# Ushio/2dGaussianSplatting

Measured on AMD Instinct MI355X. Metric: train iters/sec (fwd+bwd+Adam) + PSNR vs ref; 4K img, 1M splats, higher is better.
Workload: dtype f32; 1 GPU; 4096x4096 synthetic RGB, 1000000 Gaussians, fp32 (BASELINE.json configs[3]); width=4096, height=4096, n_splats=1000000, parallelism=rowslab1, rebin_interval=0, exchange_requested=none, exchange=none

## Files before the change

### 2dgaussiansplatting_amd/csrc/s2d_api.hip

```cpp
#include "../../include/splat2d.h"
#include "../../include/splat2d_test.h"

#include <algorithm>
#include <vector>
#include <climits>
#include <cmath>
#include <cstdarg>
#include <cstddef>
#include <cstdio>
#include <cstring>
#include <cstdlib>
#include <new>

#include "s2d_device.h"
#include "s2d_density.h"
#include "s2d_lists.h"
#include "s2d_owned.h"
#include "s2d_state.h"

using namespace s2d;

struct s2d_ctx {
    s2d_config cfg{};
    Geometry g{};
    int n = 0;
    int device = 0;
    hipStream_t stream = nullptr;
    bool own_stream = false;
    float lr = 0.05f;

    SplatState state;
    DevBuf<float> d_grads_own;
    float* d_grads = nullptr;
    DevBuf<ProjRec> d_proj;
    DevBuf<TileRect> d_rects;
    DevBuf<uint32_t> d_counts;
    DevBuf<uint32_t> d_offsets;
    DevBuf<uint32_t> d_scan_temp;
    TileLists lists;
    DevBuf<unsigned long long> d_wave_masks;
    DevBuf<uint32_t> d_exec_list;
    DevBuf<uint32_t> d_tile_exec;
    DevBuf<uint32_t> d_retire_hint;
    bool deterministic = false;
    DevBuf<float> d_det_data;
    DevBuf<uint32_t> d_det_stamp;
    DevBuf<uint32_t> d_det_touched;
    uint32_t det_epoch = 0;
    bool ref_order = false;
    uint64_t ref_max_bytes = 32ull << 30;
    DevBuf<float> d_ref_terms;
    DevBuf<float> d_pixel_sqerr;
    uint64_t chunk_pairs = 1ull << 30;
    std::vector<int> chunks;
    int chunks_used = 0;
    int chunk_built = -1;
    DevBuf<float4> d_state;
    DevBuf<uint32_t> d_chunk_alive;
    HostBuf<uint32_t> h_chunk_alive;
    bool lists_valid = false;
    bool proj_fresh = false;
    Event ev_flag;
    int check_seq = 1;
    HostBuf<int> h_rebin_stamp;
    int rebin_interval = 1;
    int since_rebin = 0;
    float margin = 0.0f;
    DevBuf<uint8_t> d_image0;
    DevBuf<uint8_t> d_ref;
    bool half_images = false;
    size_t pixel_bytes = sizeof(float4);
    SqerrTrace trace;
    DensityStats density;
    DevBuf<DeviceStatus> d_status;
    DevBuf<PairCounters> d_counters;
    HostBuf<DeviceStatus> h_status;

    float beta1t = 1.0f, beta2t = 1.0f;
    int iterations = 0;
    float good_beta1t = 1.0f, good_beta2t = 1.0f;
    int good_iterations = 0;
    bool have_target = false;
    bool have_forward = false;
    bool have_backward = false;
    char err[512] = {0};
    S2D_LOCAL ~s2d_ctx() = default;
};

namespace {

int fail(s2d_ctx* c, int code, const char* fmt, ...)
{
    if (c) {
        va_list ap;
        va_start(ap, fmt);
        vsnprintf(c->err, sizeof(c->err), fmt, ap);
        va_end(ap);
    }
    return code;
}

#define S2D_HIP(c, expr)                                                                              \
    do {                                                                                              \
        hipError_t e_ = (expr);                                                                       \
        if (e_ != hipSuccess)                                                                         \
            return fail((c), S2D_E_HIP, "%s failed: %s (%s:%d)", #expr, hipGetErrorString(e_), __FILE__, __LINE__); \
    } while (0)

struct IdleAtExit {
    hipStream_t stream;
    ~IdleAtExit() { (void)hipStreamSynchronize(stream); }
};

int use_device(s2d_ctx* c)
{
    S2D_HIP(c, hipSetDevice(c->device));
    return S2D_OK;
}

int ensure_pair_capacity(s2d_ctx* c, uint64_t need)
{
    if (need <= c->lists.capacity()) return S2D_OK;
    if (need >= 0xFFFF0000ull) return fail(c, S2D_E_NOMEM, "tile lists need %llu pairs (> 2^32)", (unsigned long long)need);
    uint64_t cap = std::max<uint64_t>(need + need / 4 + 4096, 1 << 16);
    if (cap > 0xFFFF0000ull) cap = 0xFFFF0000ull;
    if (c->ref_order) {
        const uint64_t per_slot = (uint64_t)kRefTermsStride * sizeof(float);
        if (cap * per_slot > c->ref_max_bytes) cap = std::max<uint64_t>(need, 1 << 16);
        if (cap * per_slot > c->ref_max_bytes)
            return fail(c, S2D_E_NOMEM, "the term scratch of S2D_CFG_REFERENCE_ORDER needs %llu bytes for %llu (tile, splat) pairs, "
                        "S2D_REFERENCE_ORDER_MAX_BYTES allows %llu", (unsigned long long)(cap * per_slot), (unsigned long long)cap,
                        (unsigned long long)c->ref_max_bytes);
    }
    S2D_HIP(c, hipStreamSynchronize(c->stream));
    c->lists.release_pairs();
    c->d_wave_masks.release(), c->d_exec_list.release(), c->d_det_data.release(), c->d_det_stamp.release();
    c->d_ref_terms.release();
    S2D_HIP(c, c->lists.alloc_pairs(cap));
    const auto hand_over = [&]() -> int {
        S2D_HIP(c, c->d_wave_masks.alloc((size_t)cap * 4));
        S2D_HIP(c, c->d_exec_list.alloc((size_t)cap));
        if (c->deterministic) S2D_HIP(c, c->d_det_data.alloc((size_t)cap * kDetStride));
        if (c->ref_order) S2D_HIP(c, c->d_ref_terms.alloc((size_t)cap * kRefTermsStride));
        if (c->deterministic || c->ref_order) {
            S2D_HIP(c, c->d_det_stamp.alloc((size_t)cap));
            S2D_HIP(c, hipMemsetAsync(c->d_det_stamp, 0, (size_t)cap * sizeof(uint32_t), c->stream));
        }
        return S2D_OK;
    };
    const int rc = hand_over();
    if (rc != S2D_OK) c->lists.release_pairs();
    return rc;
}

int rebuild_lists(s2d_ctx* c, int first = 0, int count = -1, bool* need_ranges = nullptr)
{
    const int n = count < 0 ? c->n : count;
    uint64_t total = 0;
    c->lists_valid = false;
    S2D_HIP(c, c->lists.count(ListInput{c->d_rects + first, c->d_counts + first, c->d_offsets + first, first, n, c->d_scan_temp},
                              c->stream, &total));
    if (need_ranges) *need_ranges = total > c->chunk_pairs;
    if (need_ranges && *need_ranges) return S2D_OK;
    if (total >= 0xFFFF0000ull)
        return fail(c, S2D_E_NOMEM, "the tile lists of splats %d..%d need more than 2^32 - 65536 (tile, splat) pairs", first, first + n - 1);
    if (int rc = ensure_pair_capacity(c, total)) return rc;
    S2D_HIP(c, c->lists.finish(c->stream));
    c->lists_valid = count < 0;
    c->since_rebin = 0;
    return S2D_OK;
}

RasterArgs raster_args(const s2d_ctx* c, int first = 0, int count = -1)
{
    RasterArgs a;
    a.tile_off = c->lists.tile_off(); a.list = c->lists.list(); a.wave_masks = c->d_wave_masks;
    a.exec_list = c->d_exec_list; a.tile_exec = c->d_tile_exec; a.retire_hint = c->d_retire_hint;
    a.proj = c->d_proj + first; a.grads = c->d_grads + (size_t)first * 9;
    a.image0 = c->d_image0; a.image_ref = c->d_ref; a.tile_sqerr = c->trace.tile_sqerr();
    a.g = c->g; a.status = c->d_status; a.iteration = c->iterations; a.counters = c->d_counters;
    a.state = c->d_state; a.any_alive = c->d_chunk_alive;
    if (c->deterministic)
        a.det = DetGather{c->d_rects + first, c->d_offsets + first, c->d_counts + first, c->d_det_data, c->d_det_stamp,
                          c->d_det_touched + first, 0u, count < 0 ? c->n : count};
    a.half_images = c->half_images; a.count = (c->cfg.flags & S2D_CFG_COUNT_PAIRS) != 0; a.exact_exp = (c->cfg.flags & S2D_CFG_EXACT_EXP) != 0;
    return a;
}

ProjectArgs project_args(const s2d_ctx* c, const float* splats, int mode)
{
    ProjectArgs a;
    a.splats = splats; a.held = c->state.held(); a.n = c->n; a.g = c->g; a.mode = mode; a.proj = c->d_proj; a.counts = c->d_counts;
    a.check = ContainmentCheck{c->d_rects, c->d_status, mode ? c->check_seq : 0, mode ? (int*)c->h_rebin_stamp : nullptr};
    if (mode == 0) a.margin = c->margin, a.row_counts = c->lists.row_counts();
    return a;
}

AdamArgs adam_args(s2d_ctx* c, uint32_t flags, bool project)
{
    const SplatState::AdamStep st = c->state.adam_step();
    AdamArgs a;
    a.splats = st.arrays.splats; a.adams = st.arrays.adams; a.grads = c->d_grads; a.compact = st.compact;
    a.held_ids = st.held_ids; a.held_count = st.held_count; a.dormant = st.dormant; a.n = c->n; a.g = c->g;
    a.beta1t = c->beta1t; a.beta2t = c->beta2t; a.lr = c->lr; a.iteration = c->iterations;
    a.mode = ((flags & S2D_STEP_OPTIMIZE_OPACITY) ? 1 : 0) | ((c->cfg.flags & S2D_CFG_ADAM_FP32) ? 2 : 0);
    a.proj = project ? (ProjRec*)c->d_proj : nullptr;
    a.check = ContainmentCheck{c->d_rects, c->d_status, c->check_seq, c->h_rebin_stamp};
    a.sq = c->trace.take_for_adam();
    return a;
}

void with_backward_walk(s2d_ctx* c, RasterArgs& a, bool need_opacity_grad)
{
    a.need_opacity_grad = need_opacity_grad;
    if (c->deterministic) a.det.now = ++c->det_epoch;
}

int plan_chunks(s2d_ctx* c)
{
    std::vector<uint32_t> cnt((size_t)c->n);
    S2D_HIP(c, hipMemcpyAsync(cnt.data(), c->d_counts, cnt.size() * sizeof(uint32_t), hipMemcpyDeviceToHost, c->stream));
    S2D_HIP(c, hipStreamSynchronize(c->stream));
    c->chunks.assign(1, 0);
    uint64_t acc = 0;
    for (int i = 0; i < c->n; i++) {
        if (acc > 0 && acc + cnt[(size_t)i] > c->chunk_pairs) {
            c->chunks.push_back(i);
            acc = 0;
        }
        acc += cnt[(size_t)i];
    }
    c->chunks.push_back(c->n);
    if (!c->d_state) S2D_HIP(c, c->d_state.alloc((size_t)c->g.W * (size_t)(c->g.row_end - c->g.row_begin)));
    if (!c->d_chunk_alive) S2D_HIP(c, c->d_chunk_alive.alloc(1));
    S2D_HIP(c, c->h_chunk_alive.alloc(1, hipHostMallocDefault));
    return S2D_OK;
}

int build_chunk(s2d_ctx* c, int k, RasterArgs* a)
{
    const int first = c->chunks[(size_t)k], count = c->chunks[(size_t)k + 1] - first;
    if (c->chunk_built != k) {
        c->chunk_built = -1;
        if (int rc = rebuild_lists(c, first, count)) return rc;
        c->chunk_built = k;
    }
    *a = raster_args(c, first, count); a->first = k == 0;
    return S2D_OK;
}

int chunked_forward(s2d_ctx* c)
{
    const int K = (int)c->chunks.size() - 1;
    c->chunks_used = 0;
    c->chunk_built = -1;
    for (int k = 0; k < K; k++) {
        RasterArgs a;
        if (int rc = build_chunk(c, k, &a)) return rc;
        S2D_HIP(c, hipMemsetAsync(c->d_chunk_alive, 0, sizeof(uint32_t), c->stream));
        S2D_HIP(c, launch_raster(RasterPass::ForwardRange, a, c->stream));
        c->chunks_used = k + 1;
        if (k + 1 < K) {
            S2D_HIP(c, hipMemcpyAsync(c->h_chunk_alive, c->d_chunk_alive, sizeof(uint32_t), hipMemcpyDeviceToHost, c->stream));
            S2D_HIP(c, hipStreamSynchronize(c->stream));
            if (*(volatile uint32_t*)c->h_chunk_alive == 0u) break;
        }
    }
    return S2D_OK;
}

int chunked_backward(s2d_ctx* c, bool need_opacity_grad, const float4* upstream = nullptr)
{
    for (int k = 0; k < c->chunks_used; k++) {
        RasterArgs a;
        if (int rc = build_chunk(c, k, &a)) return rc;
        a.upstream = upstream;
        with_backward_walk(c, a, need_opacity_grad);
        S2D_HIP(c, launch_raster(RasterPass::BackwardRange, a, c->stream));
    }
    return S2D_OK;
}

struct RasterJob {
    bool fused = false;
    bool need_opacity_grad = true;
    bool write_image = true;
};

int launch_job(s2d_ctx* c, bool optimistic, const RasterJob& job)
{
    RasterArgs a = raster_args(c);
    a.abort_stamp = optimistic ? c->check_seq : 0;
    if (job.fused) {
        with_backward_walk(c, a, job.need_opacity_grad);
        a.write_image = job.write_image;
        if (c->trace.plan(true, true) == SqerrBy::PassItself) a.sq = c->trace.job(c->iterations);
    }
    if (c->ref_order && a.exact_exp)
        S2D_HIP(c, launch_reference_forward_exact(a, c->stream));
    else
        S2D_HIP(c, launch_raster(job.fused ? RasterPass::Fused : RasterPass::Forward, a, c->stream));
    return S2D_OK;
}

enum class Stale { Frames, Projection, Lists };

void invalidate(s2d_ctx* c, Stale reach)
{
    c->have_forward = c->have_backward = false;
    if (reach >= Stale::Projection) c->proj_fresh = false;
    if (reach >= Stale::Lists) c->lists_valid = false;
}

constexpr DeviceStatus kFreshStatus{0, INT_MAX, 0, 0};

int splats_replaced(s2d_ctx* c)
{
    S2D_HIP(c, c->state.written(true));
    S2D_HIP(c, hipMemcpyAsync(c->d_status, &kFreshStatus, sizeof(DeviceStatus), hipMemcpyHostToDevice, c->stream));
    invalidate(c, Stale::Lists);
    return S2D_OK;
}

int queue_project(s2d_ctx* c, int mode)
{
    SplatState::Arrays now;
    S2D_HIP(c, c->state.current(&now));
    S2D_HIP(c, launch_project(project_args(c, now.splats, mode), c->stream));
    return S2D_OK;
}

int queue_raster(s2d_ctx* c, const RasterJob& job)
{
    if (!c->have_target) return fail(c, S2D_E_STATE, "no target image set (s2d_set_target)");
    const bool scheduled = !c->lists_valid || c->rebin_interval <= 1 || c->since_rebin >= c->rebin_interval;
    bool rebuild = scheduled;
    bool stored_image0 = !job.fused || job.write_image;
    if (!scheduled) {
        if (!c->proj_fresh) {
            c->check_seq++;
            if (int rc = queue_project(c, 1)) return rc;
            S2D_HIP(c, hipEventRecord(c->ev_flag, c->stream));
            c->proj_fresh = true;
        }
        if (int rc = launch_job(c, true, job)) return rc;
        S2D_HIP(c, hipEventSynchronize(c->ev_flag));
        rebuild = *(volatile int*)c->h_rebin_stamp == c->check_seq;
    }
    if (rebuild) {
        int rc = queue_project(c, 0);
        if (rc != S2D_OK) return rc;
        c->chunks.clear();
        bool need_ranges = false;
        if ((rc = rebuild_lists(c, 0, -1, &need_ranges)) != S2D_OK) return rc;
        if (need_ranges && (c->cfg.flags & S2D_CFG_COUNT_PAIRS))
            return fail(c, S2D_E_NOMEM, "pair counting (S2D_CFG_COUNT_PAIRS) is not available for scenes beyond %llu (tile, splat) pairs",
                        (unsigned long long)c->chunk_pairs);
        if (need_ranges && c->ref_order)
            return fail(c, S2D_E_NOMEM, "reference order (S2D_CFG_REFERENCE_ORDER) is not available for scenes beyond %llu (tile, splat) pairs",
                        (unsigned long long)c->chunk_pairs);
        c->proj_fresh = true;
        c->check_seq++;
        if (need_ranges) {
            if ((rc = plan_chunks(c)) != S2D_OK) return rc;
            if ((rc = chunked_forward(c)) != S2D_OK) return rc;
            if (job.fused && (rc = chunked_backward(c, job.need_opacity_grad)) != S2D_OK) return rc;
            stored_image0 = true;
        } else if ((rc = launch_job(c, false, job)) != S2D_OK) {
            return rc;
        }
    }
    c->have_forward = stored_image0;
    c->have_backward = false;
    return S2D_OK;
}

int queue_forward(s2d_ctx* c) { return queue_raster(c, RasterJob{}); }

int backward_queued(s2d_ctx* c, SqerrBy by)
{
    c->have_backward = true;
    S2D_HIP(c, c->trace.record(c->iterations, by));
    return S2D_OK;
}

int queue_backward_reference(s2d_ctx* c, bool need_opacity_grad, const float4* upstream)
{
    RasterArgs a = raster_args(c);
    a.upstream = upstream;
    a.need_opacity_grad = need_opacity_grad;
    SplatState::Arrays now;
    S2D_HIP(c, c->state.current(&now));
    RefOrder ro;
    ro.splats = now.splats; ro.rects = c->d_rects; ro.offsets = c->d_offsets; ro.counts = c->d_counts; ro.n = c->n;
    ro.terms = c->d_ref_terms; ro.stamp = c->d_det_stamp; ro.capacity = (uint32_t)c->lists.capacity(); ro.now = ++c->det_epoch;
    ro.pixel_sqerr = c->d_pixel_sqerr;
    S2D_HIP(c, launch_reference_backward(a, ro, c->stream));
    if (upstream) return backward_queued(c, SqerrBy::NoLoss);
    S2D_HIP(c, launch_reference_sqerr(c->d_pixel_sqerr, (size_t)c->g.W * (size_t)(c->g.row_end - c->g.row_begin),
                                      c->trace.job(c->iterations).out, c->d_status, c->iterations, c->stream));
    return backward_queued(c, SqerrBy::PassItself);
}

int density_refused(s2d_ctx* c)
{
    if ((c->cfg.flags & (S2D_CFG_COUNT_PAIRS | S2D_CFG_EXACT_EXP)) || c->ref_order)
        return fail(c, S2D_E_INVALID, "density statistics are not available with S2D_CFG_COUNT_PAIRS, S2D_CFG_EXACT_EXP or "
                    "S2D_CFG_REFERENCE_ORDER");
    return S2D_OK;
}

int queue_backward(s2d_ctx* c, bool need_opacity_grad, const float4* upstream = nullptr, bool density = false)
{
    if (!c->have_forward) return fail(c, S2D_E_STATE, "the backward pass needs s2d_forward on the current parameters");
    if (c->ref_order) return queue_backward_reference(c, need_opacity_grad, upstream);
    if (density && !c->chunks.empty())
        return fail(c, S2D_E_NOMEM, "density statistics are not available for scenes beyond %llu (tile, splat) pairs (index-range rendering)",
                    (unsigned long long)c->chunk_pairs);
    if (!c->chunks.empty()) {
        if (int rc = chunked_backward(c, need_opacity_grad, upstream)) return rc;
    } else {
        RasterArgs a = raster_args(c);
        a.upstream = upstream;
        if (density) S2D_HIP(c, c->density.next_pass(&a.density));
        with_backward_walk(c, a, need_opacity_grad);
        S2D_HIP(c, launch_raster(RasterPass::Backward, a, c->stream));
    }
    return backward_queued(c, upstream ? SqerrBy::NoLoss : c->trace.plan(false, false));
}

int queue_forward_backward(s2d_ctx* c, bool need_opacity_grad, bool write_image)
{
    if ((c->cfg.flags & S2D_CFG_COUNT_PAIRS) || c->ref_order) {
        if (int rc = queue_forward(c)) return rc;
        return queue_backward(c, need_opacity_grad);
    }
    RasterJob job;
    job.fused = true;
    job.need_opacity_grad = need_opacity_grad;
    job.write_image = write_image;
    if (int rc = queue_raster(c, job)) return rc;
    return backward_queued(c, c->trace.plan(true, c->chunks.empty()));
}

int queue_adam(s2d_ctx* c, uint32_t flags)
{
    c->beta1t *= kAdamBeta1;
    c->beta2t *= kAdamBeta2;
    const bool fuse = c->lists_valid && c->rebin_interval > 1;
    if (fuse) c->check_seq++;
    S2D_HIP(c, launch_adam(adam_args(c, flags, fuse), c->stream));
    if (fuse) S2D_HIP(c, hipEventRecord(c->ev_flag, c->stream));
    invalidate(c, Stale::Projection);
    c->proj_fresh = fuse;
    c->iterations++;
    c->since_rebin++;
    return S2D_OK;
}

int queue_status_read(s2d_ctx* c)
{
    S2D_HIP(c, hipMemcpyAsync(c->h_status, c->d_status, sizeof(DeviceStatus), hipMemcpyDeviceToHost, c->stream));
    return S2D_OK;
}

int judge_status(s2d_ctx* c)
{
    if (c->h_status->nonfinite) {
        const int k = c->h_status->first_nonfinite_iter;
        if (k >= c->good_iterations && k < c->iterations) {
            float b1 = c->good_beta1t, b2 = c->good_beta2t;
            for (int i = c->good_iterations; i <= k; i++) { b1 *= kAdamBeta1; b2 *= kAdamBeta2; }
            c->beta1t = b1;
            c->beta2t = b2;
            c->iterations = k + 1;
            invalidate(c, Stale::Frames);
        }
        return fail(c, S2D_E_NONFINITE, "non-finite parameter after iteration %d (the reference abort()s, main.cpp:752-785)", k);
    }
    c->good_beta1t = c->beta1t;
    c->good_beta2t = c->beta2t;
    c->good_iterations = c->iterations;
    return S2D_OK;
}

int check_status(s2d_ctx* c)
{
    if (int rc = queue_status_read(c)) return rc;
    S2D_HIP(c, hipStreamSynchronize(c->stream));
    return judge_status(c);
}

double mse_norm(const s2d_ctx* c) { return (double)((long long)c->g.H * c->g.W * 3); }

size_t slab_pixels(const s2d_ctx* c) { return (size_t)c->g.W * (size_t)(c->g.row_end - c->g.row_begin); }

}

extern "C" {

int s2d_abi_version(void) { return S2D_ABI_VERSION; }

int s2d_create(const s2d_config* cfg, s2d_ctx** out)
{
    if (!cfg || !out || cfg->struct_size != sizeof(s2d_config)) return S2D_E_INVALID;
    *out = nullptr;
    if (cfg->width <= 0 || cfg->height <= 0 || cfg->n_splats < 0 || cfg->width > 65536 || cfg->height > 65536)
        return S2D_E_INVALID;
    int rb = cfg->row_begin, re = cfg->row_end;
// ... 702 lines not shown
```

### 2dgaussiansplatting_amd/csrc/s2d_device.h

```cpp
#pragma once

#include <hip/hip_runtime.h>
#include <stdint.h>

#include "s2d_math.h"

namespace s2d {

struct alignas(16) ProjRec {
    float4 q0, q1, q2, q3;
};
static_assert(sizeof(ProjRec) == 64, "ProjRec must be 64 bytes");

struct TileRect {
    uint16_t tx0, tx1, ty0, ty1;
};

struct Geometry {
    int W, H;
    int row_begin;
    int row_end;
    int tiles_x;
    int trow0;
    int tiles_y;
    int num_tiles;
};

struct PairCounters {
    unsigned long long fwd_visited, fwd_active, bwd_visited, bwd_active, fwd_staged, bwd_staged, fwd_wave_execs,
        bwd_wave_execs;
    unsigned long long bwd_lane_hist[65];
    unsigned long long fwd_staged_hit;
    unsigned long long fwd_rows_hit;
    unsigned long long bwd_quadrant_execs;
};

struct DeviceStatus {
    int nonfinite;
    int first_nonfinite_iter;
    int rebin_needed;
    int pad;
};

struct SqerrJob {
    const double* tile_sqerr;
    int num_tiles;
    double* out;
    double* scratch;
};

#if defined(__HIPCC__)
__device__ __forceinline__ float as_f(int v) { return __int_as_float(v); }

__device__ __forceinline__ void raise_rebin(DeviceStatus* status, int stamp, int* host_stamp)
{
    __hip_atomic_store(&status->rebin_needed, stamp, __ATOMIC_RELAXED, __HIP_MEMORY_SCOPE_AGENT);
    if (host_stamp) __hip_atomic_store(host_stamp, stamp, __ATOMIC_RELAXED, __HIP_MEMORY_SCOPE_SYSTEM);
}

__device__ __forceinline__ ProjRec pack_proj(const Projected& p)
{
    ProjRec rec;
    rec.q0 = make_float4(p.pos_x, p.pos_y, p.a, p.b);
    rec.q1 = make_float4(p.d, p.col_r, p.col_g, p.col_b);
    rec.q2 = make_float4(p.opacity, as_f(p.begY), as_f(p.endY), p.cosT);
    const float sx2 = p.sx * p.sx, sy2 = p.sy * p.sy;
    rec.q3 = make_float4(p.sinT, 1.0f / (sx2 * p.sx), 1.0f / (sy2 * p.sy), (sx2 - sy2) / (sx2 * p.sy * p.sy));
    return rec;
}

__device__ __forceinline__ bool tile_rect_of(const Projected& p, const Geometry& g, float margin, TileRect* r)
{
    const int m = (int)margin;
    long long y0 = (long long)p.begY - m, y1 = (long long)p.endY + m;
    if (p.begY == (int)0x80000000u || p.endY == (int)0x80000000u) return false;
    if (y0 < g.row_begin) y0 = g.row_begin;
    if (y1 > g.row_end - 1) y1 = g.row_end - 1;
    if (y0 > y1) return false;
    float xlo = p.pos_x - p.hx - 1.0f - margin;
    float xhi = p.pos_x + p.hx + 1.0f + margin;
    if (!(xlo <= xhi)) return false;
    if (xhi < 0.0f || xlo > (float)(g.W - 1)) return false;
    xlo = fmaxf(xlo, 0.0f);
    xhi = fminf(xhi, (float)(g.W - 1));
    r->tx0 = (uint16_t)((int)xlo >> 4);
    r->tx1 = (uint16_t)((int)xhi >> 4);
    r->ty0 = (uint16_t)(((int)y0 >> 4) - g.trow0);
    r->ty1 = (uint16_t)(((int)y1 >> 4) - g.trow0);
    return true;
}

__device__ __forceinline__ bool rect_still_covers(const Projected& p, const Geometry& g, const TileRect& binned)
{
    TileRect r;
    if (!tile_rect_of(p, g, 0.0f, &r)) return true;
    return binned.tx0 <= binned.tx1 && r.tx0 >= binned.tx0 && r.tx1 <= binned.tx1 && r.ty0 >= binned.ty0 &&
           r.ty1 <= binned.ty1;
}
#endif

constexpr float kAnisoMargin = 1.0f;
constexpr int kRasterBatch = 64;
constexpr int kSortItemsPerThread = 16;
constexpr int kSortBlock = 256;
constexpr int kSortItemsPerBlock = kSortBlock * kSortItemsPerThread;
constexpr int kScanItemsPerThread = 8;
constexpr int kScanBlock = 256;
constexpr int kScanItemsPerBlock = kScanBlock * kScanItemsPerThread;

size_t scan_temp_words(int64_t n);
hipError_t exclusive_scan_u32(const uint32_t* in, uint32_t* out, int64_t n, uint32_t* temp, uint32_t* total_dev,
                              hipStream_t stream, uint32_t* total_host_mapped = nullptr);
size_t sort_temp_words(int64_t n);
hipError_t sort_pairs_u32(uint32_t* keys_a, uint32_t* vals_a, uint32_t* keys_b, uint32_t* vals_b, int64_t n,
                          int key_bits, uint32_t* temp, uint32_t** keys_out, uint32_t** vals_out, uint32_t* tile_first,
                          hipStream_t stream);
size_t tile_first_temp_words(int num_keys);
hipError_t launch_tile_offsets_from_first(const uint32_t* tile_first, int num_keys, uint32_t total, uint32_t* temp,
                                          uint32_t* tile_off, hipStream_t stream);

struct ContainmentCheck {
    TileRect* rects = nullptr;
    DeviceStatus* status = nullptr;
    int stamp = 0;
    int* host_stamp = nullptr;
};

struct ProjectArgs {
    const float* splats = nullptr;
    const uint8_t* held = nullptr;
    int n = 0;
    Geometry g{};
    float margin = 0.0f;
    int mode = 0;
    ProjRec* proj = nullptr;
    uint32_t* counts = nullptr;
    uint32_t* row_counts = nullptr;
    ContainmentCheck check{};
};
hipError_t launch_project(const ProjectArgs& a, hipStream_t stream);
hipError_t launch_emit_row_entries(const TileRect* rects, const uint32_t* row_offsets, const uint32_t* row_counts, int n,
                                   uint32_t* keys, uint32_t* vals, uint32_t capacity, hipStream_t stream);
hipError_t launch_emit_pairs(const TileRect* rects, const uint32_t* offsets, const uint32_t* counts, int n, Geometry g,
                             uint32_t* keys, uint32_t* vals, uint32_t capacity, hipStream_t stream);
hipError_t launch_tile_offsets(const uint32_t* sorted_keys, uint32_t num_pairs, int num_tiles,
                               uint32_t* tile_off, hipStream_t stream, uint32_t key_mask = 0xFFFFFFFFu);

constexpr int kTlMaxColumns = 512;
constexpr int kTlRowBits = 12;
size_t tl_workspace_words(uint64_t entries, int tiles_x, int tiles_y);
hipError_t launch_tile_lists_from_rows(const uint32_t* entries, const uint32_t* entry_keys, uint64_t num_entries, const uint32_t* row_off,
                                       Geometry g, uint32_t* chunk_base, uint32_t* workspace, uint32_t* tile_off, uint32_t* list,
                                       hipStream_t stream);

constexpr int kDetStride = 12;
struct DetGather {
    const TileRect* rects;
    const uint32_t* offsets;
    const uint32_t* counts;
    float* data;
    uint32_t* stamp;
    uint32_t* touched;
    uint32_t now;
    int n;
};
enum class RasterPass {
    Forward,
    Backward,
    Fused,
    ForwardRange,
    BackwardRange,
};
struct RasterArgs {
    const uint32_t* tile_off = nullptr;
    const uint32_t* list = nullptr;
    const ProjRec* proj = nullptr;
    void* image0 = nullptr;
    const void* image_ref = nullptr;
    const float4* upstream = nullptr;
    float* density = nullptr;
    unsigned long long* wave_masks = nullptr;
    uint32_t* exec_list = nullptr;
    uint32_t* tile_exec = nullptr;
    uint32_t* retire_hint = nullptr;
    float* grads = nullptr;
    double* tile_sqerr = nullptr;
    Geometry g{};
    const DeviceStatus* status = nullptr;
    int iteration = 0;
    int abort_stamp = 0;
    PairCounters* counters = nullptr;
    float4* state = nullptr;
    bool first = false;
    uint32_t* any_alive = nullptr;
    bool write_image = false;
    SqerrJob sq{};
    DetGather det{};
    bool half_images = false;
    bool count = false;
    bool exact_exp = false;
    bool need_opacity_grad = false;
};
hipError_t launch_raster(RasterPass pass, const RasterArgs& a, hipStream_t stream);
constexpr int kRefTermsStride = 9 * kTile * kTile;
struct RefOrder {
    const float* splats = nullptr;
    const TileRect* rects = nullptr;
    const uint32_t* offsets = nullptr;
    const uint32_t* counts = nullptr;
    int n = 0;
    float* terms = nullptr;
    uint32_t* stamp = nullptr;
    uint32_t capacity = 0;
    uint32_t now = 0;
    float* pixel_sqerr = nullptr;
};
hipError_t launch_reference_backward(const RasterArgs& a, const RefOrder& ro, hipStream_t stream);
hipError_t launch_reference_forward_exact(const RasterArgs& a, hipStream_t stream);
hipError_t launch_reference_sqerr(const float* pixel_sqerr, size_t pixels, double* out, const DeviceStatus* status, int iteration,
                                  hipStream_t stream);
hipError_t launch_halo_masks(const float* splats, const uint8_t* held, int n, int world, const int* row_bounds, float margin,
                             uint32_t* masks, hipStream_t stream);
hipError_t launch_halo_commit(const uint32_t* masks, int n, int rank, uint8_t* held, uint32_t* ids, uint32_t* count_dev,
                              uint32_t* scan_work, uint32_t* scan_temp, hipStream_t stream);
hipError_t launch_compact_copy(float* base, int w, const uint32_t* ids, const uint32_t* count_dev, int n, float* compact, bool to_compact,
                               hipStream_t stream);
hipError_t launch_rows_gather(const float* base, int w, const int* ids, int count, int n, float* out, hipStream_t stream);
hipError_t launch_rows_scatter(float* base, int w, const int* ids, int count, int n, const float* in, hipStream_t stream);
hipError_t launch_grads_combine(float* grads, const int* rows, int n_rows, const int* src, int world, const float* recv,
                                int n, hipStream_t stream);
constexpr int kSqerrChunks = 64;
constexpr int kSqerrScratchDoubles = kSqerrChunks + 1;
constexpr int kSqerrSmallTiles = 1024;


#if defined(__HIPCC__)
__device__ __forceinline__ double block_sum_256(double v, double* s)
{
#pragma unroll
    for (int d = 32; d >= 1; d >>= 1) v += __shfl_down(v, d, 64);
    if ((threadIdx.x & 63) == 0) s[threadIdx.x >> 6] = v;
    __syncthreads();
    const double r = ((s[0] + s[1]) + s[2]) + s[3];
    __syncthreads();
    return r;
}

__device__ __forceinline__ double sqerr_sum_small(const double* tile_sqerr, int num_tiles, double* s4)
{
    double a = 0.0;
    for (int i = (int)threadIdx.x; i < num_tiles; i += 256)
        a += __hip_atomic_load(tile_sqerr + i, __ATOMIC_RELAXED, __HIP_MEMORY_SCOPE_AGENT);
    return block_sum_256(a, s4);
}

__device__ __forceinline__ void sqerr_reduce(const double* __restrict__ tile_sqerr, int num_tiles, double* __restrict__ out,
                                             double* scratch, int first_chunk, int chunk_stride)
{
    __shared__ double s[4];
    __shared__ bool last;
    if (num_tiles <= kSqerrSmallTiles) {
        if (first_chunk != 0) return;
        const double total = sqerr_sum_small(tile_sqerr, num_tiles, s);
        if (threadIdx.x == 0) *out = total;
        return;
    }
    unsigned long long* ticket = reinterpret_cast<unsigned long long*>(scratch + kSqerrChunks);
    const int chunk = (num_tiles + kSqerrChunks - 1) / kSqerrChunks;
    unsigned long long mine = 0;
    for (int b = first_chunk; b < kSqerrChunks; b += chunk_stride, mine++) {
        const int beg = b * chunk, end = min(beg + chunk, num_tiles);
        double a0 = 0, a1 = 0, a2 = 0, a3 = 0;
        for (int i = beg + (int)threadIdx.x; i < end; i += 1024) {
            a0 += tile_sqerr[i];
            if (i + 256 < end) a1 += tile_sqerr[i + 256];
            if (i + 512 < end) a2 += tile_sqerr[i + 512];
            if (i + 768 < end) a3 += tile_sqerr[i + 768];
        }
        const double part = block_sum_256((a0 + a1) + (a2 + a3), s);
        if (threadIdx.x == 0) __hip_atomic_store(scratch + b, part, __ATOMIC_RELAXED, __HIP_MEMORY_SCOPE_AGENT);
    }
    if (threadIdx.x == 0) {
        __threadfence();
        last = mine != 0 && atomicAdd(ticket, mine) + mine == (unsigned long long)kSqerrChunks;
    }
    __syncthreads();
    if (!last) return;
    __threadfence();
    const double p = threadIdx.x < kSqerrChunks
                         ? __hip_atomic_load(scratch + threadIdx.x, __ATOMIC_RELAXED, __HIP_MEMORY_SCOPE_AGENT)
                         : 0.0;
    const double total = block_sum_256(p, s);
    if (threadIdx.x == 0) {
        *out = total;
        *ticket = 0ull;
    }
}
#endif
hipError_t launch_sqerr_finalize(SqerrJob sq, const DeviceStatus* status, int iteration, hipStream_t stream);

hipError_t launch_init_splats(float* splats, float* adams, int n, int W, int H, hipStream_t stream);
struct AdamArgs {
    float* splats = nullptr;
    float* adams = nullptr;
    float* grads = nullptr;
    const uint32_t* held_ids = nullptr;
    const uint32_t* held_count = nullptr;
    int n = 0;
    Geometry g{};
    float beta1t = 1.0f, beta2t = 1.0f, lr = 0.0f;
    int mode = 0;
    int iteration = 0;
    ProjRec* proj = nullptr;
    ContainmentCheck check{};
    uint8_t* dormant = nullptr;
    SqerrJob sq{};
    bool compact = false;
};
hipError_t launch_adam(const AdamArgs& a, hipStream_t stream);
hipError_t launch_synthetic_target(void* image_ref, bool half_images, int W, int H, int row_begin, int row_end, hipStream_t stream);
hipError_t launch_convert_f32_to_f16(const float4* src, void* dst, size_t pixels, hipStream_t stream);
hipError_t launch_convert_f16_to_f32(const void* src, float4* dst, size_t pixels, hipStream_t stream);
hipError_t launch_test_sincos(const float* x, int n, float* s, float* c, hipStream_t stream);

}
```

### 2dgaussiansplatting_amd/csrc/s2d_optim.hip

```cpp
#include <hip/hip_fp16.h>

#include "s2d_device.h"

namespace s2d {

__global__ __launch_bounds__(256) void init_splats_kernel(float* __restrict__ splats, float* __restrict__ adams, int n,
                                                          int W, int H)
{
    const int i = blockIdx.x * blockDim.x + threadIdx.x;
    if (i >= n) return;
    const Splat s = init_splat((uint32_t)i, W, H);
    float* o = splats + (size_t)i * 9;
    o[0] = s.pos_x; o[1] = s.pos_y; o[2] = s.sx; o[3] = s.sy; o[4] = s.rot;
    o[5] = s.col_r; o[6] = s.col_g; o[7] = s.col_b; o[8] = s.opacity;
    float* a = adams + (size_t)i * 18;
#pragma unroll
    for (int k = 0; k < 18; k++) a[k] = 0.0f;
}

__device__ __forceinline__ bool finite_f32(float x) { return (f32_bits(x) & 0x7f800000u) != 0x7f800000u; }

__device__ __forceinline__ void adam_update_one(float (&v)[9], float (&mv)[18], const float (&gr)[9], int W, int H, float beta1t,
                                                float beta2t, float lr, int mode, int iteration, DeviceStatus* status)
{
#pragma unroll
    for (int k = 0; k < 9; k++)
        if (k < 8 || (mode & 1))
            v[k] = adam_optimize(mv[2 * k], mv[2 * k + 1], v[k], gr[k], lr, beta1t, beta2t, (mode & 2) != 0);
    v[0] = glm_clamp(v[0], 0.0f, (float)W - 1.0f);
    v[1] = glm_clamp(v[1], 0.0f, (float)H - 1.0f);
    v[2] = glm_clamp(v[2], 1.0f, 1024.0f);
    v[3] = glm_clamp(v[3], 1.0f, 1024.0f);
    v[5] = glm_clamp(v[5], 0.0f, 1.0f);
    v[6] = glm_clamp(v[6], 0.0f, 1.0f);
    v[7] = glm_clamp(v[7], 0.0f, 1.0f);
    v[8] = glm_clamp(v[8], 0.1f, 1.0f);
    const bool ok = finite_f32(v[5]) && finite_f32(v[6]) && finite_f32(v[7]) && finite_f32(v[2]) &&
                    finite_f32(v[3]) && finite_f32(v[4]) && finite_f32(v[0]);
    if (!ok) {
        atomicOr(&status->nonfinite, 1);
        atomicMin(&status->first_nonfinite_iter, iteration);
    }
}

__device__ __forceinline__ void project_updated(const float (&v)[9], int i, const Geometry& g, DeviceStatus* status,
                                                ProjRec* __restrict__ proj, const TileRect* __restrict__ rects,
                                                int check_stamp, int* __restrict__ host_stamp)
{
    const float reach = 3.0f * fmaxf(v[2], v[3]) + 2.0f;
    if (v[1] + reach < (float)g.row_begin || v[1] - reach > (float)g.row_end) {
        proj[i].q2 = make_float4(v[8], as_f(1), as_f(0), 0.0f);
        return;
    }
    Splat s;
    s.pos_x = v[0]; s.pos_y = v[1]; s.sx = v[2]; s.sy = v[3]; s.rot = v[4];
    s.col_r = v[5]; s.col_g = v[6]; s.col_b = v[7]; s.opacity = v[8];
    const Projected p = project(s);
    proj[i] = pack_proj(p);
    if (!rect_still_covers(p, g, rects[i])) raise_rebin(status, check_stamp, host_stamp);
}

__device__ __forceinline__ bool adam_prologue(const DeviceStatus* status, int iteration, const SqerrJob& sq)
{
    if (status->first_nonfinite_iter < iteration) return false;
    if (sq.tile_sqerr != nullptr && blockIdx.x < (unsigned)kSqerrChunks)
        sqerr_reduce(sq.tile_sqerr, sq.num_tiles, sq.out, sq.scratch, (int)blockIdx.x, min((int)gridDim.x, kSqerrChunks));
    return true;
}

template <int WIDTH>
__device__ __forceinline__ void lds_fill(float* lds, const float* __restrict__ src, const uint32_t* s_ids, int base, int cnt)
{
    const int floats = cnt * WIDTH;
    if (s_ids == nullptr) {
        const float* p = src + (size_t)base * WIDTH;
        const int vec = floats >> 2;
        for (int q = threadIdx.x; q < vec; q += 256) reinterpret_cast<float4*>(lds)[q] = reinterpret_cast<const float4*>(p)[q];
        for (int q = (vec << 2) + threadIdx.x; q < floats; q += 256) lds[q] = p[q];
    } else {
        for (int q = threadIdx.x; q < floats; q += 256) lds[q] = src[(size_t)s_ids[q / WIDTH] * WIDTH + q % WIDTH];
    }
}

template <int WIDTH>
__device__ __forceinline__ void lds_drain(float* __restrict__ dst, const float* lds, const uint32_t* s_ids, int base, int cnt)
{
    const int floats = cnt * WIDTH;
    if (s_ids == nullptr) {
        float* p = dst + (size_t)base * WIDTH;
        const int vec = floats >> 2;
        for (int q = threadIdx.x; q < vec; q += 256) reinterpret_cast<float4*>(p)[q] = reinterpret_cast<const float4*>(lds)[q];
        for (int q = (vec << 2) + threadIdx.x; q < floats; q += 256) p[q] = lds[q];
    } else {
        for (int q = threadIdx.x; q < floats; q += 256) dst[(size_t)s_ids[q / WIDTH] * WIDTH + q % WIDTH] = lds[q];
    }
}

__global__ __launch_bounds__(256) void adam_kernel(float* __restrict__ splats, float* __restrict__ adams,
                                                   float* __restrict__ grads, const uint32_t* __restrict__ held_ids,
                                                   const uint32_t* __restrict__ held_count, int n, Geometry g,
                                                   float beta1t, float beta2t, float lr, int mode, int iteration,
                                                   DeviceStatus* __restrict__ status, ProjRec* __restrict__ proj,
                                                   const TileRect* __restrict__ rects, int check_stamp,
                                                   int* __restrict__ host_stamp, uint8_t* __restrict__ dormant, SqerrJob sq,
                                                   int compact)
{
    __shared__ __attribute__((aligned(16))) float buf[256 * 18];
    __shared__ uint32_t s_idbuf[256];
    if (!adam_prologue(status, iteration, sq)) return;
    const int total = held_ids ? (int)min(*held_count, (uint32_t)n) : n;
    const int base = blockIdx.x * 256, cnt = min(256, total - base), t = threadIdx.x;
    if (cnt <= 0) return;
    const bool mine = t < cnt;
    const uint32_t* s_ids = nullptr;
    int i = base + t;
    if (held_ids) {
        if (mine) {
            i = (int)held_ids[base + t];
            s_idbuf[t] = (uint32_t)i;
        }
        s_ids = s_idbuf;
        __syncthreads();
    }
    const uint32_t* const s_ids_state = compact ? nullptr : s_ids;
    float v[9], mv[18], gr[9];
    lds_fill<9>(buf, grads, s_ids, base, cnt);
    __syncthreads();
#pragma unroll
    for (int k = 0; k < 9; k++) gr[k] = mine ? buf[t * 9 + k] : 0.0f;
    bool live = false;
    if (mine) {
#pragma unroll
        for (int k = 0; k < 9; k++) live = live || (f32_bits(gr[k]) != 0u);
        if (!live) live = dormant == nullptr || dormant[i] == 0;
    }
    if (!__syncthreads_or(live)) return;
    for (int q = t; q < 256 * 9 / 4; q += 256) reinterpret_cast<float4*>(buf)[q] = make_float4(0.f, 0.f, 0.f, 0.f);
    __syncthreads();
    lds_drain<9>(grads, buf, s_ids, base, cnt);
    __syncthreads();
    lds_fill<9>(buf, splats, s_ids_state, base, cnt);
    __syncthreads();
#pragma unroll
    for (int k = 0; k < 9; k++) v[k] = mine ? buf[t * 9 + k] : 0.0f;
    __syncthreads();
    lds_fill<18>(buf, adams, s_ids_state, base, cnt);
    __syncthreads();
#pragma unroll
    for (int k = 0; k < 18; k++) mv[k] = mine ? buf[t * 18 + k] : 0.0f;
    if (mine) {
        adam_update_one(v, mv, gr, g.W, g.H, beta1t, beta2t, lr, mode, iteration, status);
        if (dormant) {
            uint32_t any = 0u;
#pragma unroll
            for (int k = 0; k < 18; k++) any |= f32_bits(mv[k]);
            dormant[i] = any == 0u ? 1 : 0;
        }
#pragma unroll
        for (int k = 0; k < 18; k++) buf[t * 18 + k] = mv[k];
    }
    __syncthreads();
    lds_drain<18>(adams, buf, s_ids_state, base, cnt);
    __syncthreads();
    if (mine) {
#pragma unroll
        for (int k = 0; k < 9; k++) buf[t * 9 + k] = v[k];
    }
    __syncthreads();
    lds_drain<9>(splats, buf, s_ids_state, base, cnt);
    if (proj && mine) project_updated(v, i, g, status, proj, rects, check_stamp, host_stamp);
}

__device__ __forceinline__ uint2 pack_half4(float4 c)
{
    const __half2 a = __floats2half2_rn(c.x, c.y), b = __floats2half2_rn(c.z, c.w);
    uint2 v;
    v.x = *reinterpret_cast<const uint32_t*>(&a);
    v.y = *reinterpret_cast<const uint32_t*>(&b);
    return v;
}

template <bool HALF>
__global__ __launch_bounds__(256) void synthetic_target_kernel(void* __restrict__ image_ref, int W, int H, int row_begin,
                                                               int row_end)
{
    const int x = blockIdx.x * blockDim.x + threadIdx.x;
    const int y = row_begin + (int)blockIdx.y;
    if (x >= W || y >= row_end) return;
    const float fx = (float)x / (float)W;
    const float4 c = make_float4(fx, 1.0f - fx, (float)y / (float)H, 1.0f);
    const size_t at = (size_t)(y - row_begin) * W + x;
    if (HALF) reinterpret_cast<uint2*>(image_ref)[at] = pack_half4(c);
    else reinterpret_cast<float4*>(image_ref)[at] = c;
}

__global__ __launch_bounds__(256) void convert_f32_to_f16_kernel(const float4* __restrict__ src, uint2* __restrict__ dst,
                                                                 size_t pixels)
{
    const size_t i = (size_t)blockIdx.x * blockDim.x + threadIdx.x;
    if (i < pixels) dst[i] = pack_half4(src[i]);
}

__global__ __launch_bounds__(256) void convert_f16_to_f32_kernel(const uint2* __restrict__ src, float4* __restrict__ dst,
                                                                 size_t pixels)
{
    const size_t i = (size_t)blockIdx.x * blockDim.x + threadIdx.x;
    if (i >= pixels) return;
    const uint2 v = src[i];
    const float2 a = __half22float2(*reinterpret_cast<const __half2*>(&v.x));
    const float2 b = __half22float2(*reinterpret_cast<const __half2*>(&v.y));
    dst[i] = make_float4(a.x, a.y, b.x, b.y);
}

__global__ __launch_bounds__(256) void test_sincos_kernel(const float* __restrict__ x, int n, float* __restrict__ s,
                                                          float* __restrict__ c)
{
    const int i = blockIdx.x * blockDim.x + threadIdx.x;
    if (i >= n) return;
    s[i] = sinf_ref(x[i]);
    c[i] = cosf_ref(x[i]);
}

hipError_t launch_init_splats(float* splats, float* adams, int n, int W, int H, hipStream_t stream)
{
    if (n <= 0) return hipSuccess;
    hipLaunchKernelGGL(init_splats_kernel, dim3((n + 255) / 256), dim3(256), 0, stream, splats, adams, n, W, H);
    return hipGetLastError();
}

hipError_t launch_adam(const AdamArgs& a, hipStream_t stream)
{
    if (a.n <= 0) return hipSuccess;
    hipLaunchKernelGGL(adam_kernel, dim3((a.n + 255) / 256), dim3(256), 0, stream, a.splats, a.adams, a.grads, a.held_ids,
                       a.held_count, a.n, a.g, a.beta1t, a.beta2t, a.lr, a.mode, a.iteration, a.check.status, a.proj,
                       (const TileRect*)a.check.rects, a.check.stamp, a.check.host_stamp, a.dormant, a.sq,
                       (a.compact && a.held_ids) ? 1 : 0);
    return hipGetLastError();
}

hipError_t launch_synthetic_target(void* image_ref, bool half_images, int W, int H, int row_begin, int row_end, hipStream_t stream)
{
    const dim3 grid((W + 255) / 256, row_end - row_begin);
    if (half_images)
        hipLaunchKernelGGL(synthetic_target_kernel<true>, grid, dim3(256), 0, stream, image_ref, W, H, row_begin, row_end);
    else
        hipLaunchKernelGGL(synthetic_target_kernel<false>, grid, dim3(256), 0, stream, image_ref, W, H, row_begin, row_end);
    return hipGetLastError();
}

hipError_t launch_convert_f32_to_f16(const float4* src, void* dst, size_t pixels, hipStream_t stream)
{
    if (!pixels) return hipSuccess;
    hipLaunchKernelGGL(convert_f32_to_f16_kernel, dim3((unsigned)((pixels + 255) / 256)), dim3(256), 0, stream, src,
                       reinterpret_cast<uint2*>(dst), pixels);
    return hipGetLastError();
}

hipError_t launch_convert_f16_to_f32(const void* src, float4* dst, size_t pixels, hipStream_t stream)
{
    if (!pixels) return hipSuccess;
    hipLaunchKernelGGL(convert_f16_to_f32_kernel, dim3((unsigned)((pixels + 255) / 256)), dim3(256), 0, stream,
                       reinterpret_cast<const uint2*>(src), dst, pixels);
    return hipGetLastError();
}

hipError_t launch_test_sincos(const float* x, int n, float* s, float* c, hipStream_t stream)
{
    if (n <= 0) return hipSuccess;
    hipLaunchKernelGGL(test_sincos_kernel, dim3((n + 255) / 256), dim3(256), 0, stream, x, n, s, c);
    return hipGetLastError();
}

}
```

Baseline: 628.2 iterations/s.

## Skip memory traffic for inert splats in Adam and rezero only nonzero gradients

The Adam kernel now builds a per-block liveness bitmask through wave ballots. Loads and stores of splat and moment records are skipped for splats with zero gradient whose dormant state means no update is needed, and re-projection is also skipped when the projection is known current and no containment check failed. Gradient zeroing now writes back only the lines that were nonzero, replacing the full zero-and-drain pass. This cuts global memory traffic in a bandwidth-bound optimizer step over 1M splats, at the cost of extra predicate logic. It also relies on proj_fresh and rebin-state tracking being correct.

New measurement: 636.1 iterations/s, median of 6. +1.3%, better.

```diff
diff --git a/2dgaussiansplatting_amd/csrc/s2d_api.hip b/2dgaussiansplatting_amd/csrc/s2d_api.hip
--- a/2dgaussiansplatting_amd/csrc/s2d_api.hip
+++ b/2dgaussiansplatting_amd/csrc/s2d_api.hip
@@ -205,6 +205,7 @@
     a.beta1t = c->beta1t; a.beta2t = c->beta2t; a.lr = c->lr; a.iteration = c->iterations;
     a.mode = ((flags & S2D_STEP_OPTIMIZE_OPACITY) ? 1 : 0) | ((c->cfg.flags & S2D_CFG_ADAM_FP32) ? 2 : 0);
     a.proj = project ? (ProjRec*)c->d_proj : nullptr;
+    a.proj_current = c->proj_fresh;
     a.check = ContainmentCheck{c->d_rects, c->d_status, c->check_seq, c->h_rebin_stamp};
     a.sq = c->trace.take_for_adam();
     return a;
diff --git a/2dgaussiansplatting_amd/csrc/s2d_device.h b/2dgaussiansplatting_amd/csrc/s2d_device.h
--- a/2dgaussiansplatting_amd/csrc/s2d_device.h
+++ b/2dgaussiansplatting_amd/csrc/s2d_device.h
@@ -312,6 +312,7 @@
     int mode = 0;
     int iteration = 0;
     ProjRec* proj = nullptr;
+    bool proj_current = false;
     ContainmentCheck check{};
     uint8_t* dormant = nullptr;
     SqerrJob sq{};
diff --git a/2dgaussiansplatting_amd/csrc/s2d_optim.hip b/2dgaussiansplatting_amd/csrc/s2d_optim.hip
--- a/2dgaussiansplatting_amd/csrc/s2d_optim.hip
+++ b/2dgaussiansplatting_amd/csrc/s2d_optim.hip
@@ -68,31 +68,109 @@
     return true;
 }
 
+__device__ __forceinline__ bool record_live(const uint64_t* s_live, int r)
+{
+    return s_live == nullptr || ((s_live[r >> 6] >> (r & 63)) & 1ull) != 0ull;
+}
+
 template <int WIDTH>
-__device__ __forceinline__ void lds_fill(float* lds, const float* __restrict__ src, const uint32_t* s_ids, int base, int cnt)
+__device__ __forceinline__ bool line_live(const uint64_t* s_live, int q)
+{
+    return s_live == nullptr || record_live(s_live, (4 * q) / WIDTH) || record_live(s_live, (4 * q + 3) / WIDTH);
+}
+
+template <int WIDTH>
+__device__ __forceinline__ void lds_fill(float* lds, const float* __restrict__ src, const uint32_t* s_ids, const uint64_t* s_live,
+                                         int base, int cnt)
 {
     const int floats = cnt * WIDTH;
     if (s_ids == nullptr) {
         const float* p = src + (size_t)base * WIDTH;
         const int vec = floats >> 2;
-        for (int q = threadIdx.x; q < vec; q += 256) reinterpret_cast<float4*>(lds)[q] = reinterpret_cast<const float4*>(p)[q];
-        for (int q = (vec << 2) + threadIdx.x; q < floats; q += 256) lds[q] = p[q];
+        constexpr int kLines = (256 * WIDTH / 4 + 255) / 256;
+        float4 x[kLines];
+        uint32_t take = 0u;
+#pragma unroll
+        for (int j = 0; j < kLines; j++) {
+            const int q = (int)threadIdx.x + 256 * j;
+            take |= (q < vec && line_live<WIDTH>(s_live, q) ? 1u : 0u) << j;
+        }
+#pragma unroll
+        for (int j = 0; j < kLines; j++) {
+            x[j] = make_float4(0.f, 0.f, 0.f, 0.f);
+            if ((take >> j) & 1u) x[j] = reinterpret_cast<const float4*>(p)[(int)threadIdx.x + 256 * j];
+        }
+#pragma unroll
+        for (int j = 0; j < kLines; j++)
+            if ((take >> j) & 1u) reinterpret_cast<float4*>(lds)[(int)threadIdx.x + 256 * j] = x[j];
+        for (int q = (vec << 2) + threadIdx.x; q < floats; q += 256)
+            if (record_live(s_live, q / WIDTH)) lds[q] = p[q];
     } else {
-        for (int q = threadIdx.x; q < floats; q += 256) lds[q] = src[(size_t)s_ids[q / WIDTH] * WIDTH + q % WIDTH];
+        for (int q = threadIdx.x; q < floats; q += 256)
+            if (record_live(s_live, q / WIDTH)) lds[q] = src[(size_t)s_ids[q / WIDTH] * WIDTH + q % WIDTH];
     }
 }
 
 template <int WIDTH>
-__device__ __forceinline__ void lds_drain(float* __restrict__ dst, const float* lds, const uint32_t* s_ids, int base, int cnt)
+__device__ __forceinline__ void lds_drain(float* __restrict__ dst, const float* lds, const uint32_t* s_ids, const uint64_t* s_live,
+                                          int base, int cnt)
 {
     const int floats = cnt * WIDTH;
     if (s_ids == nullptr) {
         float* p = dst + (size_t)base * WIDTH;
         const int vec = floats >> 2;
-        for (int q = threadIdx.x; q < vec; q += 256) reinterpret_cast<float4*>(p)[q] = reinterpret_cast<const float4*>(lds)[q];
-        for (int q = (vec << 2) + threadIdx.x; q < floats; q += 256) p[q] = lds[q];
+        for (int q = threadIdx.x; q < vec; q += 256)
+            if (line_live<WIDTH>(s_live, q)) reinterpret_cast<float4*>(p)[q] = reinterpret_cast<const float4*>(lds)[q];
+        for (int q = (vec << 2) + threadIdx.x; q < floats; q += 256)
+            if (record_live(s_live, q / WIDTH)) p[q] = lds[q];
     } else {
-        for (int q = threadIdx.x; q < floats; q += 256) dst[(size_t)s_ids[q / WIDTH] * WIDTH + q % WIDTH] = lds[q];
+        for (int q = threadIdx.x; q < floats; q += 256)
+            if (record_live(s_live, q / WIDTH)) dst[(size_t)s_ids[q / WIDTH] * WIDTH + q % WIDTH] = lds[q];
+    }
+}
+
+__device__ __forceinline__ uint32_t grads_fill(float* lds, const float* __restrict__ grads, const uint32_t* s_ids, int base, int cnt)
+{
+    const int floats = cnt * 9;
+    uint32_t nz = 0u;
+    int j = 0;
+    if (s_ids == nullptr) {
+        const float* p = grads + (size_t)base * 9;
+        const int vec = floats >> 2;
+        for (int q = threadIdx.x; q < vec; q += 256, j++) {
+            const float4 x = reinterpret_cast<const float4*>(p)[q];
+            reinterpret_cast<float4*>(lds)[q] = x;
+            nz |= ((f32_bits(x.x) | f32_bits(x.y) | f32_bits(x.z) | f32_bits(x.w)) != 0u ? 1u : 0u) << j;
+        }
+        for (int q = (vec << 2) + threadIdx.x; q < floats; q += 256, j++) {
+            const float x = p[q];
+            lds[q] = x;
+            nz |= (f32_bits(x) != 0u ? 1u : 0u) << j;
+        }
+    } else {
+        for (int q = threadIdx.x; q < floats; q += 256, j++) {
+            const float x = grads[(size_t)s_ids[q / 9] * 9 + q % 9];
+            lds[q] = x;
+            nz |= (f32_bits(x) != 0u ? 1u : 0u) << j;
+        }
+    }
+    return nz;
+}
+
+__device__ __forceinline__ void grads_rezero(float* __restrict__ grads, const uint32_t* s_ids, int base, int cnt, uint32_t nz)
+{
+    const int floats = cnt * 9;
+    int j = 0;
+    if (s_ids == nullptr) {
+        float* p = grads + (size_t)base * 9;
+        const int vec = floats >> 2;
+        for (int q = threadIdx.x; q < vec; q += 256, j++)
+            if ((nz >> j) & 1u) reinterpret_cast<float4*>(p)[q] = make_float4(0.f, 0.f, 0.f, 0.f);
+        for (int q = (vec << 2) + threadIdx.x; q < floats; q += 256, j++)
+            if ((nz >> j) & 1u) p[q] = 0.0f;
+    } else {
+        for (int q = threadIdx.x; q < floats; q += 256, j++)
+            if ((nz >> j) & 1u) grads[(size_t)s_ids[q / 9] * 9 + q % 9] = 0.0f;
     }
 }
 
@@ -103,11 +181,13 @@
                                                    DeviceStatus* __restrict__ status, ProjRec* __restrict__ proj,
                                                    const TileRect* __restrict__ rects, int check_stamp,
                                                    int* __restrict__ host_stamp, uint8_t* __restrict__ dormant, SqerrJob sq,
-                                                   int compact)
+                                                   int compact, int proj_current)
 {
     __shared__ __attribute__((aligned(16))) float buf[256 * 18];
     __shared__ uint32_t s_idbuf[256];
+    __shared__ uint64_t s_live_words[4];
     if (!adam_prologue(status, iteration, sq)) return;
+    const int last_failed_check = __hip_atomic_load(&status->rebin_needed, __ATOMIC_RELAXED, __HIP_MEMORY_SCOPE_AGENT);
     const int total = held_ids ? (int)min(*held_count, (uint32_t)n) : n;
     const int base = blockIdx.x * 256, cnt = min(256, total - base), t = threadIdx.x;
     if (cnt <= 0) return;
@@ -124,31 +204,34 @@
     }
     const uint32_t* const s_ids_state = compact ? nullptr : s_ids;
     float v[9], mv[18], gr[9];
-    lds_fill<9>(buf, grads, s_ids, base, cnt);
+    const bool asleep = mine && dormant != nullptr && dormant[i] != 0;
+    const uint32_t grads_nonzero = grads_fill(buf, grads, s_ids, base, cnt);
     __syncthreads();
 #pragma unroll
     for (int k = 0; k < 9; k++) gr[k] = mine ? buf[t * 9 + k] : 0.0f;
+    const bool may_skip = proj == nullptr || (proj_current != 0 && last_failed_check != check_stamp - 1);
     bool live = false;
     if (mine) {
 #pragma unroll
         for (int k = 0; k < 9; k++) live = live || (f32_bits(gr[k]) != 0u);
-        if (!live) live = dormant == nullptr || dormant[i] == 0;
-    }
+        if (!live) live = !may_skip || !asleep;
+    }
+    const uint64_t wave_live = __ballot(live);
+    if ((t & 63) == 0) s_live_words[t >> 6] = wave_live;
     if (!__syncthreads_or(live)) return;
-    for (int q = t; q < 256 * 9 / 4; q += 256) reinterpret_cast<float4*>(buf)[q] = make_float4(0.f, 0.f, 0.f, 0.f);
-    __syncthreads();
-    lds_drain<9>(grads, buf, s_ids, base, cnt);
-    __syncthreads();
-    lds_fill<9>(buf, splats, s_ids_state, base, cnt);
+    const int inert_records = cnt - (__popcll(s_live_words[0]) + __popcll(s_live_words[1]) + __popcll(s_live_words[2]) + __popcll(s_live_words[3]));
+    const uint64_t* const s_live = __builtin_amdgcn_readfirstlane(inert_records) == 0 ? nullptr : s_live_words;
+    grads_rezero(grads, s_ids, base, cnt, grads_nonzero);
+    lds_fill<9>(buf, splats, s_ids_state, s_live, base, cnt);
     __syncthreads();
 #pragma unroll
     for (int k = 0; k < 9; k++) v[k] = mine ? buf[t * 9 + k] : 0.0f;
     __syncthreads();
-    lds_fill<18>(buf, adams, s_ids_state, base, cnt);
-    __syncthreads();
-#pragma unroll
-    for (int k = 0; k < 18; k++) mv[k] = mine ? buf[t * 18 + k] : 0.0f;
-    if (mine) {
+    lds_fill<18>(buf, adams, s_ids_state, s_live, base, cnt);
+    __syncthreads();
+    if (live) {
+#pragma unroll
+        for (int k = 0; k < 18; k++) mv[k] = buf[t * 18 + k];
         adam_update_one(v, mv, gr, g.W, g.H, beta1t, beta2t, lr, mode, iteration, status);
         if (dormant) {
             uint32_t any = 0u;
@@ -160,15 +243,15 @@
         for (int k = 0; k < 18; k++) buf[t * 18 + k] = mv[k];
     }
     __syncthreads();
-    lds_drain<18>(adams, buf, s_ids_state, base, cnt);
+    lds_drain<18>(adams, buf, s_ids_state, s_live, base, cnt);
     __syncthreads();
     if (mine) {
 #pragma unroll
         for (int k = 0; k < 9; k++) buf[t * 9 + k] = v[k];
     }
     __syncthreads();
-    lds_drain<9>(splats, buf, s_ids_state, base, cnt);
-    if (proj && mine) project_updated(v, i, g, status, proj, rects, check_stamp, host_stamp);
+    lds_drain<9>(splats, buf, s_ids_state, s_live, base, cnt);
+    if (proj && live) project_updated(v, i, g, status, proj, rects, check_stamp, host_stamp);
 }
 
 __device__ __forceinline__ uint2 pack_half4(float4 c)
@@ -234,7 +317,7 @@
     hipLaunchKernelGGL(adam_kernel, dim3((a.n + 255) / 256), dim3(256), 0, stream, a.splats, a.adams, a.grads, a.held_ids,
                        a.held_count, a.n, a.g, a.beta1t, a.beta2t, a.lr, a.mode, a.iteration, a.check.status, a.proj,
                        (const TileRect*)a.check.rects, a.check.stamp, a.check.host_stamp, a.dormant, a.sq,
-                       (a.compact && a.held_ids) ? 1 : 0);
+                       (a.compact && a.held_ids) ? 1 : 0, a.proj_current ? 1 : 0);
     return hipGetLastError();
 }
 
```
